# IQTLabs/WITW

Measured on AMD Instinct MI355X. Metric: image-pairs/sec (embedding+similarity), higher is better.
Workload: dtype f32

## Files before the change

include/witw_hip.h:

```cpp
#ifndef WITW_HIP_H
#define WITW_HIP_H

#ifdef __cplusplus
extern "C" {
#endif

const char* witw_last_error(void);
int witw_version(void);
int witw_device_check(int device);
const char* witw_last_kernel_variant(void);
const char* witw_last_conv_form(void);


int witw_conv3x3_tile_n(int cout);
int witw_conv3x3_workgroup_waves(int B, int H, int W, int Cout, int stride_h);
long long witw_conv3x3_packed_floats(int cout, int cin);
int witw_conv3x3_bias_floats(int cout);
int witw_conv3x3_pack_weights(const float* w_kcrs, float* wpk, int cout, int cin, int transpose_flip, void* stream);
int witw_nchw_to_nhwc8(const float* x, float* y, int B, int C, int H, int W, void* stream);
int witw_conv3x3_fwd(const float* x, const float* wpk, const float* bias, const float* dropmask, float* y, int B, int H,
                     int W, int Cin, int Cout, int stride_h, int pad_circular, int relu, int pool, int out_nchw,
                     void* stream);

int witw_conv3x3_first_pack(const float* w, float* wf, int C, int round_bf16, void* stream);
int witw_conv_first2_bf16_fwd(const float* x, const void* wf0, const float* bias0, const void* wpk2, const float* bias2, void* y,
                              int B, int C, int H, int W, int pad_circular, void* stream);
int witw_conv_first2_bf16_fwd_train(const float* x, const void* wf0, const float* bias0, const void* wpk2, const float* bias2, void* y,
                                    unsigned char* pool_code, unsigned char* gate_bits, int B, int C, int H, int W, int pad_circular,
                                    void* stream);
int witw_conv3x3_bf16_gatebits_ok(int B, int H, int W, int Cin, int Cout);
int witw_conv3x3_bf16_fwd_gatebits(const void* x_bf16, const void* wpk_bf16, const float* bias, const void* gate_bits, void* y, int B, int H,
                                   int W, int Cin, int Cout, int pad_circular, int relu, void* stream);
int witw_conv3x3_first_fwd(const float* x, const float* wf, const float* bias, void* y, int B, int C, int H, int W,
                           int pad_circular, int relu, int out_bf16, void* stream);

int witw_conv3x3_fwd_ex(const float* x, const float* wpk, const float* bias, const float* dropmask, const float* gate,
                        const float* post_scale, const float* post_shift, float* y, unsigned char* pool_code, int B, int H,
                        int W, int Cin, int Cout, int stride_h, int pad_circular, int relu, float lrelu_slope, int pool,
                        int out_nchw, int dilate_h, void* stream);
int witw_conv3x3_dil_skip(int enable);
long long witw_conv3x3_packed_floats_wino(int cout, int cin);
int witw_conv3x3_pack_weights_wino(const float* w_kcrs, float* wpk_wino, int cout, int cin, void* stream);
int witw_conv3x3_fwd_wino(const float* x, const float* wpk, const float* wpk_wino, const float* bias, const float* dropmask,
                          const float* gate, const float* post_scale, const float* post_shift, float* y, unsigned char* pool_code,
                          int B, int H, int W, int Cin, int Cout, int stride_h, int pad_circular, int relu, float lrelu_slope,
                          int pool, int out_nchw, int dilate_h, void* stream);
int witw_conv3x3_wino(int enable);
int witw_maxpool2x2_bwd(const float* dy, const unsigned char* pool_code, float* dx, int B, int Hp, int Wp, int H, int W,
                        int C, void* stream);
int witw_nchw_to_nhwc(const float* x, float* y, int B, int C, int H, int W, int Cpad, void* stream);
int witw_conv3x3_wgrad_splits(int B, int Ho, int Wo, int Cin, int Cout);
long long witw_conv3x3_wgrad_workspace_floats(int B, int H, int W, int Cin, int Cout, int stride_h);
int witw_conv3x3_wgrad(const float* x, const float* dz, float* dw, float* db, float* workspace, int B, int H, int W, int Cin,
                       int cin_real, int Cout, int stride_h, int pad_circular, int accumulate, void* stream);
int witw_adam_step(float* param, const float* grad, float* exp_avg, float* exp_avg_sq, long long n, float lr, float beta1,
                   float beta2, float eps, int step, void* stream);
int witw_adam_step_multi(float* const* param, const float* const* grad, float* const* exp_avg, float* const* exp_avg_sq,
                         const long long* n, const int* step, int count, float lr, float beta1, float beta2, float eps, void* stream);

long long witw_match_workspace_floats(int Bo, int Bs);
int witw_match_fwd(const float* ov, const float* su, int Bo, int Bs, int We, long long* orientation, float* distance,
                   float* score, float* workspace, void* stream);
int witw_match_fwd_masked(const float* ov, const float* su, int Bo, int Bs, int We, long long* orientation, float* distance,
                          float* score, float* workspace, const unsigned long long* shift_mask, void* stream);
long long witw_match_fixed_workspace_floats(int Bo, int Bs);
int witw_match_fwd_fixed(const float* ov, const float* su, int Bo, int Bs, int We, const long long* shift ,
                         long long* orientation, float* distance, float* score, float* workspace, void* stream);
long long witw_match_spectrum_floats(long long n_embeddings);
int witw_match_spectrum(const float* emb, float* spec, int B, int W, int role ,
                        void* stream);
long long witw_match_dft_workspace_floats(int Bo, int Bs);
int witw_match_fwd_dft(const float* ov, const float* su, const float* spec_ov, const float* spec_su, int Bo, int Bs, int We,
                       long long* orientation, float* distance, float* score, float* workspace, void* stream);
int witw_match_fwd_dft_gap(const float* ov, const float* su, const float* spec_ov, const float* spec_su, int Bo, int Bs, int We,
                           long long* orientation, float* distance, float* score, float* gap, float* workspace, void* stream);
int witw_match_fwd_dft_masked(const float* ov, const float* su, const float* spec_ov, const float* spec_su, int Bo, int Bs, int We,
                              long long* orientation, float* distance, float* score, float* gap , float* workspace,
                              const unsigned long long* shift_mask, void* stream);
long long witw_match_bwd_scratch_floats(int Bo, int Bs, int We);
int witw_match_bwd(const float* ov, const float* su, const long long* orientation, const float* score, const float* workspace,
                   const float* grad_distance, float* grad_ov, float* grad_su, float* scratch, int Bo, int Bs, int We,
                   void* stream);
int witw_crop_overhead(const float* ov, const long long* orientation, float* out , int Bo, int Bs,
                       int We, void* stream);
int witw_l2_distance(const float* cropped , const float* su , float* distance, int Bo, int Bs, int n,
                     void* stream);
int witw_rank_count(const float* distance , int* ranks , int Bo, int Bs, int true_offset, void* stream);

int witw_topk_smallest(const float* distance, float* values, long long* indices, int Bo, int Bs, int k, long long row_offset,
                       void* stream);
long long witw_topk_workspace_bytes(int Bo, int Bs, int k);
int witw_topk_smallest_ws(const float* distance, float* values, long long* indices, int Bo, int Bs, int k, long long row_offset,
                          void* workspace, void* stream);
int witw_topk_smallest_after(const float* distance, float* values, long long* indices, int Bo, int Bs, int k, long long row_offset,
                             const float* after_value, const long long* after_index, void* workspace, void* stream);
int witw_rank_count_thresh(const float* distance, const float* threshold, int* ranks, int Bo, int Bs, void* stream);

int witw_match_pairs(const float* ov, const float* su, const float* wn, const float* sn, const int* pair_o, const int* pair_s,
                     int n_pairs, int Bo, int Bs, int We, long long* orientation, float* distance, float* score, void* stream);
int witw_rank_count_band(const float* distance, const float* threshold, float eps, int* counts, int* pair_o, int* pair_s,
// ... 184 lines not shown
```

witw_amd/_lib.py:

```python
import ctypes
import os
from ctypes import c_char_p, c_float, c_int, c_longlong, c_void_p

from . import build as _build

_LIB = None
_GUARDS = None

SIGNATURES = {
    'witw_last_error': (c_char_p, []),
    'witw_version': (c_int, []),
    'witw_last_kernel_variant': (c_char_p, []),
    'witw_last_conv_form': (c_char_p, []),
    'witw_device_check': (c_int, [c_int]),
    'witw_conv3x3_tile_n': (c_int, [c_int]),
    'witw_conv3x3_workgroup_waves': (c_int, [c_int] * 5),
    'witw_conv3x3_packed_floats': (c_longlong, [c_int, c_int]),
    'witw_conv3x3_bias_floats': (c_int, [c_int]),
    'witw_conv3x3_pack_weights': (c_int, [c_void_p, c_void_p, c_int, c_int, c_int, c_void_p]),
    'witw_nchw_to_nhwc8': (c_int, [c_void_p, c_void_p, c_int, c_int, c_int, c_int, c_void_p]),
    'witw_conv3x3_fwd': (c_int, [c_void_p, c_void_p, c_void_p, c_void_p, c_void_p] + [c_int] * 10 + [c_void_p]),
    'witw_conv3x3_fwd_ex': (c_int, [c_void_p] * 9 + [c_int] * 8 + [c_float] + [c_int] * 3 + [c_void_p]),
    'witw_conv3x3_dil_skip': (c_int, [c_int]),
    'witw_conv3x3_packed_floats_wino': (c_longlong, [c_int, c_int]),
    'witw_conv3x3_pack_weights_wino': (c_int, [c_void_p, c_void_p, c_int, c_int, c_void_p]),
    'witw_conv3x3_fwd_wino': (c_int, [c_void_p] * 10 + [c_int] * 8 + [c_float] + [c_int] * 3 + [c_void_p]),
    'witw_conv3x3_wino': (c_int, [c_int]),
    'witw_maxpool2x2_bwd': (c_int, [c_void_p, c_void_p, c_void_p] + [c_int] * 6 + [c_void_p]),
    'witw_conv3x3_packed_floats_taps4': (c_longlong, [c_int, c_int]),
    'witw_conv3x3_pack_weights_taps4': (c_int, [c_void_p, c_void_p, c_int, c_int, c_int, c_void_p]),
    'witw_conv3x3_fwd_taps4': (c_int, [c_void_p] * 7 + [c_int] * 6 + [c_float, c_int, c_void_p]),
    'witw_conv3x3_taps4_ksplit': (c_int, [c_int] * 5),
    'witw_conv3x3_fwd_taps4_ex': (c_int, [c_void_p] * 7 + [c_int] * 6 + [c_float] + [c_int] * 5 + [c_void_p]),
    'witw_conv3x3_wgrad_taps4': (c_int, [c_void_p] * 5 + [c_int] * 7 + [c_void_p]),
    'witw_nchw_to_nhwc': (c_int, [c_void_p, c_void_p, c_int, c_int, c_int, c_int, c_int, c_void_p]),
    'witw_conv3x3_wgrad_splits': (c_int, [c_int] * 5),
    'witw_conv3x3_wgrad_workspace_floats': (c_longlong, [c_int] * 6),
    'witw_conv3x3_wgrad': (c_int, [c_void_p] * 5 + [c_int] * 9 + [c_void_p]),
    'witw_adam_step': (c_int, [c_void_p, c_void_p, c_void_p, c_void_p, c_longlong, c_float, c_float, c_float, c_float, c_int,
                               c_void_p]),
    'witw_adam_step_multi': (c_int, [c_void_p] * 6 + [c_int, c_float, c_float, c_float, c_float, c_void_p]),
    'witw_conv3x3_first_pack': (c_int, [c_void_p, c_void_p, c_int, c_int, c_void_p]),
    'witw_conv3x3_first_fwd': (c_int, [c_void_p, c_void_p, c_void_p, c_void_p] + [c_int] * 7 + [c_void_p]),
    'witw_conv3x3_bf16_mfma16': (c_int, [c_int]),
    'witw_conv3x3_bf16_wres': (c_int, [c_int]),
    'witw_conv3x3_bf16_packed_elems': (c_longlong, [c_int, c_int]),
    'witw_conv3x3_bf16_pack_weights': (c_int, [c_void_p, c_void_p, c_int, c_int, c_void_p]),
    'witw_conv3x3_bf16_pack_weights_ex': (c_int, [c_void_p, c_void_p, c_int, c_int, c_int, c_void_p]),
    'witw_conv3x3_bf16_pack_weights_multi': (c_int, [c_void_p] * 7 + [c_int, c_void_p]),
    'witw_nchw_f32_to_nhwc_bf16': (c_int, [c_void_p, c_void_p] + [c_int] * 5 + [c_void_p]),
    'witw_conv3x3_bf16_fwd': (c_int, [c_void_p] * 4 + [c_int] * 10 + [c_void_p]),
    'witw_conv3x3_bf16_fwd_ex': (c_int, [c_void_p] * 7 + [c_int] * 11 + [c_void_p]),
    'witw_maxpool2x2_bwd_bf16': (c_int, [c_void_p] * 3 + [c_int] * 6 + [c_void_p]),
    'witw_octet_elems': (c_longlong, [c_int] * 4),
    'witw_nhwc_bf16_to_octet': (c_int, [c_void_p, c_void_p] + [c_int] * 4 + [c_void_p]),
    'witw_conv3x3_wgrad_bf16_workspace_floats': (c_longlong, [c_int] * 6),
    'witw_conv3x3_wgrad_bf16': (c_int, [c_void_p] * 5 + [c_int] * 9 + [c_void_p]),
    'witw_conv3x3_wgrad_bf16_nhwc_workspace_floats': (c_longlong, [c_int] * 6),
    'witw_conv3x3_wgrad_bf16_mfma16': (c_int, [c_int]),
    'witw_conv3x3_wgrad_bf16_nhwc': (c_int, [c_void_p] * 5 + [c_int] * 9 + [c_void_p]),
    'witw_conv3x3_f16x3_packed_elems': (c_longlong, [c_int, c_int]),
    'witw_conv3x3_f16x3_pack_weights': (c_int, [c_void_p, c_void_p, c_int, c_int, c_void_p]),
    'witw_nchw_f32_to_split_f16': (c_int, [c_void_p, c_void_p] + [c_int] * 5 + [c_void_p]),
    'witw_split_f16_to_f32': (c_int, [c_void_p, c_void_p, c_longlong, c_int, c_void_p]),
    'witw_conv3x3_f16x3_fwd': (c_int, [c_void_p] * 4 + [c_int] * 10 + [c_void_p]),
    'witw_conv3x3_f16x3_pack_weights_ex': (c_int, [c_void_p, c_void_p, c_int, c_int, c_int, c_void_p]),
    'witw_conv3x3_f16x3_fwd_ex': (c_int, [c_void_p] * 8 + [c_int] * 11 + [c_void_p]),
    'witw_maxpool2x2_bwd_split': (c_int, [c_void_p] * 3 + [c_int] * 6 + [c_void_p]),
    'witw_octet_split_elems': (c_longlong, [c_int] * 4),
    'witw_split_f16_to_octet': (c_int, [c_void_p, c_void_p] + [c_int] * 4 + [c_void_p]),
    'witw_conv3x3_wgrad_f16x3_workspace_floats': (c_longlong, [c_int] * 6),
    'witw_conv3x3_wgrad_f16x3': (c_int, [c_void_p] * 6 + [c_int] * 9 + [c_void_p]),
    'witw_conv4x4s2_first_fwd': (c_int, [c_void_p] * 6 + [c_int] * 5 + [c_float, c_void_p]),
    'witw_space_to_depth2': (c_int, [c_void_p, c_void_p] + [c_int] * 9 + [c_void_p, c_void_p, c_void_p]),
    'witw_space_to_depth2_mosaic': (c_int, [c_void_p, c_void_p] + [c_int] * 5 + [c_void_p]),
    'witw_taps4_splitk_finish': (c_int, [c_void_p, c_int, c_void_p, c_int, c_float] + [c_void_p] * 3 + [c_int] * 7 + [c_void_p]),
    'witw_gem_pool': (c_int, [c_void_p, c_void_p] + [c_int] * 8 + [c_float, c_void_p, c_void_p, c_void_p]),
    'witw_bn_workspace_floats': (c_longlong, [c_int] * 4),
    'witw_bn_train_stats': (c_int, [c_void_p] + [c_int] * 6 + [c_void_p, c_void_p, c_float, c_float] + [c_void_p] * 8),
    'witw_bn_lrelu_bwd': (c_int, [c_void_p] * 8 + [c_int] * 6 + [c_float, c_void_p, c_void_p]),
# ... 135 lines not shown
```

witw_amd/csrc/conv3x3.hip:

```cpp
#include "common.h"
#include <stdlib.h>
#include <algorithm>

namespace {

constexpr int TW_WIDE = 64;

__device__ const f32x4 g_zero_f4[1] = {{0.f, 0.f, 0.f, 0.f}};

struct ConvArgs {
    const float* x;
    const float* wpk;
    const float* bias;
    const float* dropmask;
    const float* post_scale;
    const float* post_shift;
    float lrelu;
    unsigned char* pool_code;
    const float* gate;
    float* y;
    int B, H, W, Cin, Cout;
    int Ho, Wo;
    int tiles_x, tiles_y;
    int n_tiles, sp_total, sp_per_xcd, xcd_map;
    int circ, relu, out_nchw;
    int force_nw;
    int force_geo;
    int dil_h;
    int tap_base;
    int ksplit, kc_per_split;
    size_t split_stride;
    int s2d, s2d_h, s2d_w, valid_h, valid_w;
    int wino;
    const float* wpk_wino;
#ifdef WITW_STAMPS
    unsigned long long* stamps;
#endif
};

template <int NW, bool POOL>
__device__ __forceinline__ void conv_wino_h2(const ConvArgs& p, f32x4* smem) {
    constexpr int TH = NW, TW = 64, IW = TW + 2, IH = TH + 2;
    constexpr int NTHREADS = 64 * NW;
    constexpr int WTN = 64;
    constexpr int IN_F4 = 2 * IH * IW;
    constexpr int W_F4 = 12 * 2 * WTN;
    constexpr int STAGE_F4 = IN_F4 + W_F4;
    constexpr int NIN = (IN_F4 + NTHREADS - 1) / NTHREADS;
    constexpr int NWT = W_F4 / NTHREADS;
    static_assert(NWT * NTHREADS == W_F4, "the filter slab splits evenly over the workgroup");

    const int tid = threadIdx.x;
    const int lane = tid & 63;
    const int wave = tid >> 6;
    const int l31 = lane & 31;
    const int hq = lane >> 5;

    int ntile, sp;
    if (p.xcd_map) {
        const int g = blockIdx.x >> 3;
        ntile = g % p.n_tiles;
        sp = (blockIdx.x & 7) * p.sp_per_xcd + g / p.n_tiles;
        if (sp >= p.sp_total) return;
    } else {
        ntile = blockIdx.x / p.sp_total;
        sp = blockIdx.x - ntile * p.sp_total;
    }
    const int tiles_img = p.tiles_x * p.tiles_y;
    const int b = sp / tiles_img;
    sp -= b * tiles_img;
    const int ty = sp / p.tiles_x;
    const int tx = sp - ty * p.tiles_x;
    const int oy0 = ty * TH;
    const int ox0 = tx * TW;
    const int n0 = ntile * WTN;
    const int nkc = p.Cin >> 3;

    constexpr unsigned OOR = 0x80000000u;
    const size_t img_floats = (size_t)p.H * p.W * p.Cin;
    __amdgpu_buffer_rsrc_t in_rs = __builtin_amdgcn_make_buffer_rsrc((void*)(p.x + (size_t)b * img_floats), 0,
                                                                     (unsigned)(img_floats * 4), 0x00020000);
    __amdgpu_buffer_rsrc_t w_rs = __builtin_amdgcn_make_buffer_rsrc(
        (void*)(reinterpret_cast<const f32x4*>(p.wpk_wino) + (size_t)ntile * nkc * W_F4), 0, (unsigned)nkc * W_F4 * 16u, 0x00020000);
    unsigned gin[NIN];
#pragma unroll
    for (int i = 0; i < NIN; ++i) {
        const int s = tid + i * NTHREADS;
        const int pix = s >> 1, q = s & 1;
        const int r = pix / IW, c = pix - r * IW;
        const int gr = oy0 - 1 + r;
        int gc = ox0 - 1 + c;
        bool ok = (s < IN_F4) && gr >= 0 && gr < p.H;
        if (p.circ) {
            gc %= p.W;
            if (gc < 0) gc += p.W;
        } else {
            ok = ok && gc >= 0 && gc < p.W;
        }
        gin[i] = ok ? (unsigned)((((size_t)gr * p.W + gc) * p.Cin + q * 4) * 4) : OOR;
    }
    const unsigned gwoff = (unsigned)tid * 16u;
    f32x4 rin[NIN], rw[NWT];
    auto load_one = [&](int kc, int i) {
        if (i < NIN) rin[i] = __builtin_bit_cast(f32x4, __builtin_amdgcn_raw_buffer_load_b128(in_rs, gin[i], (unsigned)kc * 32u, 0));
        else rw[i - NIN] = __builtin_bit_cast(f32x4, __builtin_amdgcn_raw_buffer_load_b128(
                 w_rs, gwoff, (unsigned)kc * W_F4 * 16u + (unsigned)(i - NIN) * (NTHREADS * 16u), 0));
    };
    auto store_one = [&](int buf, int i) {
        f32x4* in_s = smem + buf * STAGE_F4;
        if (i < NIN) {
            const int s = tid + i * NTHREADS;
            f32x4* dst = (NIN * NTHREADS == IN_F4 || s < IN_F4) ? in_s + (s & 1) * (IH * IW) + (s >> 1) : smem + 2 * STAGE_F4;
            *dst = rin[i];
        } else {
            in_s[IN_F4 + tid + (i - NIN) * NTHREADS] = rw[i - NIN];
        }
    };

    const int wm = wave >> 1, wn = wave & 1;
    const int abase = hq * (IH * IW) + 2 * wm * IW + l31;
    const int wbase = hq * WTN + wn * 32 + l31;
    f32x16 acc[4][2];
#pragma unroll
    for (int t = 0; t < 4; ++t)
#pragma unroll
        for (int ct = 0; ct < 2; ++ct)
#pragma unroll
            for (int r = 0; r < 16; ++r) acc[t][ct][r] = 0.f;

    f32x4 fa[2][4], fb[2][4];
    auto read_a = [&](int set, const f32x4* in_s, int s, int i) { fa[set][i] = in_s[abase + i * IW + 32 * (s & 1) + (s >> 1)]; };
    auto read_b = [&](int set, const f32x4* w_s, int kw, int t) { fb[set][t] = w_s[(kw * 4 + t) * 2 * WTN + wbase]; };
    auto transform2 = [&](int set, int k) {
        const int j = k >> 1;
        const float d0 = fa[set][0][j], d1 = fa[set][1][j], d2 = fa[set][2][j], d3 = fa[set][3][j];
        if ((k & 1) == 0) {
            fa[set][0][j] = d0 - d2;
            fa[set][3][j] = d1 - d3;
        } else {
            fa[set][1][j] = d1 + d2;
            fa[set][2][j] = d2 - d1;
        }
    };
    auto mfma_one = [&](int set, int bset, int ct, int i) {
        const int j = i >> 2, t = i & 3;
        acc[t][ct] = __builtin_amdgcn_mfma_f32_32x32x2f32(fa[set][t][j], fb[bset][t][j], acc[t][ct], 0, 0, 0);
    };

#pragma unroll
    for (int i = 0; i < NIN + NWT; ++i) load_one(0, i);
#pragma unroll
    for (int i = 0; i < NIN + NWT; ++i) store_one(0, i);
    __syncthreads();
#pragma unroll
    for (int i = 0; i < 4; ++i) read_b(0, smem + IN_F4, 0, i);
    __builtin_amdgcn_sched_barrier(0);
#pragma unroll
    for (int i = 0; i < 4; ++i) read_a(0, smem, 0, i);
#pragma unroll
    for (int k = 0; k < 8; ++k) transform2(0, k);

    auto step = [&](int set, int bset, int ct, auto&& mem, bool barrier_mid) {
#pragma unroll
        for (int i = 0; i < 16; ++i) {
            mfma_one(set, bset, ct, i);
            mem(i);
            if (i >= 8) transform2(set ^ 1, i - 8);
            __builtin_amdgcn_sched_barrier(0);
            if (barrier_mid && i == 7) {
                __syncthreads();
                __builtin_amdgcn_sched_barrier(0);
            }
        }
    };
    static_assert(16 - 6 - (NIN + NWT) >= 0, "step too short to hide the staging instructions");

    for (int kc = 0; kc < nkc; ++kc) {
        const int cur = kc & 1;
        const int kn = (kc + 1 < nkc) ? kc + 1 : kc;
        const f32x4* in_s = smem + cur * STAGE_F4;
        const f32x4* w_s = in_s + IN_F4;
        const f32x4* in_n = smem + (cur ^ 1) * STAGE_F4;
        step(0, 0, 0, [&](int i) {
            if (i < 4) read_a(1, in_s, 1, i);
            else if (i < 6) read_b(1, w_s, 1, i - 4);
            else if (i < 6 + NIN + NWT) load_one(kn, i - 6);
        }, false);
        step(1, 0, 1, [&](int i) {
            if (i < 4) read_a(0, in_s, 2, i);
            else if (i < 6) read_b(1, w_s, 1, i - 2);
        }, false);
        step(0, 1, 0, [&](int i) {
            if (i < 4) read_a(1, in_s, 3, i);
            else if (i < 8) read_b(0, w_s, 2, i - 4);
        }, false);
        step(1, 1, 1, [&](int i) {
            if (i < 4) read_a(0, in_s, 4, i);
            else if (i < 4 + NIN + NWT) store_one(cur ^ 1, i - 4);
        }, false);
        step(0, 0, 0, [&](int i) {
            if (i < 4) read_a(1, in_s, 5, i);
        }, true);
        step(1, 0, 1, [&](int i) {
            if (i < 4) read_a(0, in_n, 0, i);
            else if (i < 8) read_b(1, in_n + IN_F4, 0, i - 4);
        }, false);
#pragma unroll
        for (int t = 0; t < 4; ++t) fb[0][t] = fb[1][t];
    }

    f32x16 yv[2][2];
#pragma unroll
    for (int ct = 0; ct < 2; ++ct)
#pragma unroll
        for (int r = 0; r < 16; ++r) {
            const float m0 = acc[0][ct][r], m1 = acc[1][ct][r], m2 = acc[2][ct][r], m3 = acc[3][ct][r];
            yv[0][ct][r] = (m0 + m1) + m2;
            yv[1][ct][r] = (m1 - m2) - m3;
        }
    const int nb = n0 + wn * 32;
    const int nch = nb + l31;
    const float bv = p.bias[nch];
    const float dm = (p.dropmask != nullptr && nch < p.Cout) ? p.dropmask[(size_t)b * p.Cout + nch] : 1.f;
    const int act = p.relu;
    auto fin = [&](float v) {
        v = (v + bv) * dm;
        if (act == 1) v = fmaxf(v, 0.f);
        else if (act == 2) v = v > 0.f ? v : v * p.lrelu;
        return v;
    };
    const int Hy = POOL ? (p.Ho >> 1) : p.Ho;
    const int Wy = POOL ? (p.Wo >> 1) : p.Wo;
    float* slab = reinterpret_cast<float*>(smem) + wave * (32 * 32);
    const int prow = lane >> 3, pc4 = (lane & 7) * 4;
    if constexpr (!POOL) {
#pragma unroll
        for (int k = 0; k < 2; ++k)
#pragma unroll
            for (int ct = 0; ct < 2; ++ct) {
#pragma unroll
                for (int r = 0; r < 16; ++r) slab[((r & 3) + 8 * (r >> 2) + 4 * hq) * 32 + l31] = fin(yv[k][ct][r]);
                const int yy = oy0 + 2 * wm + k;
#pragma unroll
                for (int g = 0; g < 4; ++g) {
                    const int m = g * 8 + prow;
                    const f32x4 v = *reinterpret_cast<const f32x4*>(slab + m * 32 + pc4);
                    const int xx = ox0 + 32 * ct + m;
                    if (yy < Hy && xx < Wy && nb + pc4 < p.Cout)
                        __builtin_nontemporal_store(v, reinterpret_cast<f32x4*>(p.y + (((size_t)b * Hy + yy) * Wy + xx) * p.Cout + nb + pc4));
                }
            }
    } else {
        const int yy = (oy0 + 2 * wm) >> 1;
#pragma unroll
        for (int ct = 0; ct < 2; ++ct)
#pragma unroll
            for (int g = 0; g < 4; ++g)
#pragma unroll
                for (int e = 0; e < 2; ++e) {
                    const int r = 4 * g + 2 * e;
                    const float a00 = yv[0][ct][r], a01 = yv[0][ct][r + 1], a10 = yv[1][ct][r], a11 = yv[1][ct][r + 1];
                    const float m = fmaxf(fmaxf(a00, a01), fmaxf(a10, a11));
                    const int pc = 16 * ct + 4 * g + 2 * hq + e;
                    slab[pc * 32 + l31] = fin(m);
                    const int xx = (ox0 >> 1) + pc;
                    if (p.pool_code != nullptr && yy < Hy && xx < Wy && nch < p.Cout) {
                        const int code = (a00 == m) ? 0 : (a01 == m) ? 1 : (a10 == m) ? 2 : 3;
                        p.pool_code[(((size_t)b * Hy + yy) * Wy + xx) * p.Cout + nch] = (unsigned char)code;
                    }
                }
#pragma unroll
        for (int g = 0; g < 4; ++g) {
            const int pc = g * 8 + prow;
            const f32x4 v = *reinterpret_cast<const f32x4*>(slab + pc * 32 + pc4);
            const int xx = (ox0 >> 1) + pc;
            if (yy < Hy && xx < Wy && nb + pc4 < p.Cout)
                __builtin_nontemporal_store(v, reinterpret_cast<f32x4*>(p.y + (((size_t)b * Hy + yy) * Wy + xx) * p.Cout + nb + pc4));
        }
    }
}

template <int TN, int SH, bool POOL, int NW, int GEO, int TAPS = 9>
__global__ __launch_bounds__(64 * NW) void conv3x3_nhwc_f32_kernel(ConvArgs p) {
    static_assert(TAPS == 9 || TAPS == 4, "3x3 window or a 2x2 sub-window");
    constexpr bool NARROW = GEO == 1;
    constexpr bool DIL = GEO == 2;
    static_assert(!DIL || (TN == 128 && NW == 8 && SH == 1 && TAPS == 9 && !POOL), "the dilated form exists for the 8-wave 128-channel tile");
    constexpr int TH = NARROW ? 4 * NW : NW;
    constexpr int TW = NARROW ? 16 : 64;
    constexpr int IW = TW + 2;
    constexpr int NTHREADS = 64 * NW;
    constexpr int IH = (TH - 1) * SH + 3;
    constexpr int IN_F4 = 2 * IH * IW;
    constexpr int W_F4 = TAPS * 2 * TN;
    constexpr int STAGE_F4 = IN_F4 + W_F4;
    constexpr int NIN = (IN_F4 + NTHREADS - 1) / NTHREADS;
    constexpr int NWT = (W_F4 + NTHREADS - 1) / NTHREADS;
    constexpr int WGM = (TN == 128) ? NW / 2 : NW;
    constexpr int WM = (2 * NW) / WGM;
    constexpr int WN = 2;

    constexpr bool WINO = SH == 1 && TAPS == 9 && GEO == 0 && (TN == 128 || POOL);
    constexpr int WINO_F4 = WINO ? 2 * (2 * (NW + 2) * IW + 12 * 2 * 64) + 1 : 0;
    constexpr int DIRECT_F4 = (2 * STAGE_F4 + 1 > NW * 512) ? 2 * STAGE_F4 + 1 : NW * 512;
    constexpr int SMEM_F4 = DIRECT_F4 > WINO_F4 ? DIRECT_F4 : WINO_F4;
    __shared__ f32x4 smem[SMEM_F4];
    static_assert(SMEM_F4 * 16 >= NW * 32 * 64 * 4, "the buffer must hold one epilogue slab per wave");
    if constexpr (WINO) {
        if (p.wino) {
            conv_wino_h2<NW, POOL>(p, smem);
            return;
        }
    }

    const int tid = threadIdx.x;
    const int lane = tid & 63;
    const int wave = tid >> 6;
    const int l31 = lane & 31;
    const int hq = lane >> 5;

    int ntile, sp;
    if (p.xcd_map) {
        const int g = blockIdx.x >> 3;
        ntile = g % p.n_tiles;
        sp = (blockIdx.x & 7) * p.sp_per_xcd + g / p.n_tiles;
        if (sp >= p.sp_total) return;
    } else {
        ntile = blockIdx.x / p.sp_total;
        sp = blockIdx.x - ntile * p.sp_total;
    }
    const int tiles_img = p.tiles_x * p.tiles_y;
    const int b = sp / tiles_img;
    sp -= b * tiles_img;
    const int ty = sp / p.tiles_x;
    const int tx = sp - ty * p.tiles_x;
    const int oy0 = ty * TH;
    const int ox0 = tx * TW;
    const int n0 = ntile * TN;
    int nkc = p.Cin >> 3;
    int kc_lo = 0;
    if constexpr (TAPS == 4) {
        if (p.ksplit > 1) {
            kc_lo = (int)blockIdx.y * p.kc_per_split;
            nkc = min(nkc - kc_lo, p.kc_per_split);
        }
    }

    constexpr unsigned OOR = 0x80000000u;
    const int Hp = p.dil_h ? (p.H - 1) / 2 + 1 : p.H;
    const size_t img_floats = (size_t)Hp * p.W * p.Cin;
    __amdgpu_buffer_rsrc_t in_rs = __builtin_amdgcn_make_buffer_rsrc(
        (void*)(p.x + (size_t)b * img_floats + (size_t)kc_lo * 8), 0, (unsigned)(img_floats * 4) - (unsigned)kc_lo * 32u, 0x00020000);
    const unsigned wtile_bytes = (unsigned)nkc * W_F4 * 16u;
    __amdgpu_buffer_rsrc_t w_rs = __builtin_amdgcn_make_buffer_rsrc(
        (void*)(reinterpret_cast<const f32x4*>(p.wpk) + ((size_t)ntile * (p.Cin >> 3) + kc_lo) * W_F4), 0, wtile_bytes, 0x00020000);
    unsigned gin[NIN];
#pragma unroll
    for (int i = 0; i < NIN; ++i) {
        const int s = tid + i * NTHREADS;
        const int pix = s >> 1, q = s & 1;
        const int r = pix / IW, c = pix - r * IW;
        const int gr = oy0 * SH - 1 + r;
// ... 419 lines not shown
                v[j] = w[(((size_t)ci * src_cin + co) * 3 + (2 - kh)) * 3 + (2 - kw)];
        }
    }
    reinterpret_cast<f32x4*>(wpk)[idx] = v;
}

__global__ void pack_weights_wino_kernel(const float* __restrict__ w, float* __restrict__ wpk, int Cout, int Cin, int nkc,
                                         size_t total) {
    const size_t idx = (size_t)blockIdx.x * blockDim.x + threadIdx.x;
    if (idx >= total) return;
    size_t t = idx;
    const int n = t % 64; t /= 64;
    const int q = t % 2; t /= 2;
    const int tr = t % 4; t /= 4;
    const int kw = t % 3; t /= 3;
    const int kc = t % nkc; t /= nkc;
    const int co = (int)t * 64 + n;
    f32x4 v = {0.f, 0.f, 0.f, 0.f};
#pragma unroll
    for (int j = 0; j < 4; ++j) {
        const int ci = kc * 8 + q * 4 + j;
        if (co < Cout && ci < Cin) {
            const float* g = w + ((size_t)co * Cin + ci) * 9 + kw;
            const float g0 = g[0], g1 = g[3], g2 = g[6];
            v[j] = tr == 0 ? g0 : tr == 1 ? ((g0 + g1) + g2) * 0.5f : tr == 2 ? ((g0 - g1) + g2) * 0.5f : g2;
        }
    }
    reinterpret_cast<f32x4*>(wpk)[idx] = v;
}

__global__ void nchw_to_nhwc8_kernel(const float* __restrict__ x, float* __restrict__ y, int B, int C, int H, int W) {
    const size_t npix = (size_t)B * H * W;
    const size_t idx = (size_t)blockIdx.x * blockDim.x + threadIdx.x;
    if (idx >= npix) return;
    const size_t hw = (size_t)H * W;
    const size_t b = idx / hw, r = idx - b * hw;
    float v[8];
#pragma unroll
    for (int c = 0; c < 8; ++c) v[c] = (c < C) ? x[(b * C + c) * hw + r] : 0.f;
    f32x4* o = reinterpret_cast<f32x4*>(y + idx * 8);
    o[0] = f32x4{v[0], v[1], v[2], v[3]};
    o[1] = f32x4{v[4], v[5], v[6], v[7]};
}

__global__ void nchw_to_nhwc_kernel(const float* __restrict__ x, float* __restrict__ y, int C, int Cp, size_t hw, size_t total) {
    const size_t idx = (size_t)blockIdx.x * blockDim.x + threadIdx.x;
    if (idx >= total) return;
    const int c = idx % Cp;
    const size_t t = idx / Cp;
    const size_t b = t / hw, r = t - b * hw;
    y[idx] = (c < C) ? x[(b * C + c) * hw + r] : 0.f;
}

template <int TN, int SH, bool POOL, int NW, int GEO, int TAPS = 9>
int launch_conv_nw(ConvArgs a, hipStream_t st) {
    a.tiles_y = cdiv(a.Ho, GEO == 1 ? 4 * NW : NW);
    a.tiles_x = cdiv(a.Wo, GEO == 1 ? 16 : 64);
    const long long sp_total = (long long)a.B * a.tiles_x * a.tiles_y;
    a.n_tiles = cdiv(a.Cout, a.wino ? 64 : TN);
    a.sp_per_xcd = (int)((sp_total + 7) / 8);
    if (sp_total < 8) a.xcd_map = 0;
    const long long grid = a.xcd_map ? 8LL * a.sp_per_xcd * a.n_tiles : sp_total * a.n_tiles;
    if (grid <= 0 || grid > 0x7fffffffLL || sp_total > 0x7fffffffLL) {
        witw_set_error("conv3x3: grid %lld out of range", grid);
        return WITW_ERR_INVALID;
    }
    a.sp_total = (int)sp_total;
    const unsigned gy = (TAPS == 4 && a.ksplit > 1) ? (unsigned)a.ksplit : 1u;
    hipLaunchKernelGGL((conv3x3_nhwc_f32_kernel<TN, SH, POOL, NW, GEO, TAPS>), dim3((unsigned)grid, gy), dim3(64 * NW), 0, st, a);
    WITW_CHECK_LAUNCH("conv3x3_nhwc_f32");
    witw_note_variant("conv3x3_nhwc_f32_kernel<%d,%d,%s,%d,%d,%d>", TN, SH, POOL ? "true" : "false", NW, GEO, TAPS);
    if (a.wino) witw_note_conv_form("wino_h2");
    return WITW_OK;
}

int choose_waves(int B, int Ho, int Wo, int Cout, int force_nw) {
    const int TN = (Cout >= 128) ? 128 : 64;
    const long long big = (long long)cdiv(Cout, TN) * B * cdiv(Wo, TW_WIDE) * cdiv(Ho, 8);
    if (force_nw == 4) return 4;
    return (force_nw == 8 || ((Ho % 8) == 0 && witw_fills_rounds(big))) ? 8 : 4;
}

bool choose_narrow(int Wo, int force_geo) { return force_geo == 1 || (force_geo != 0 && Wo <= 32); }

int env_int(const char* name, int dflt) {
    const char* e = getenv(name);
    return e ? atoi(e) : dflt;
}

int g_dil_skip = -1;
int dil_skip() {
    if (g_dil_skip < 0) {
        const char* e = getenv("WITW_CONV_DILSKIP");
        g_dil_skip = e ? (atoi(e) != 0) : 1;
    }
    return g_dil_skip;
}

int g_wino = -1;
int wino_on() {
    if (g_wino < 0) {
        const char* e = getenv("WITW_CONV_WINO");
        g_wino = e ? (atoi(e) != 0) : 1;
    }
    return g_wino;
}

template <int TN, int SH, bool POOL>
int launch_conv(ConvArgs a, hipStream_t st) {
    const bool wino = SH == 1 && (TN == 128 || POOL) && a.wpk_wino != nullptr && wino_on() && a.gate == nullptr && !a.dil_h &&
                      !a.out_nchw && a.post_scale == nullptr && (a.Cout & 3) == 0 && a.force_geo != 1 &&
                      !choose_narrow(a.Wo, a.force_geo);
    a.wino = wino ? 1 : 0;
    if (wino) return choose_waves(a.B, a.Ho, a.Wo, a.Cout, a.force_nw) == 8 ? launch_conv_nw<TN, SH, POOL, 8, 0>(a, st)
                                                                          : launch_conv_nw<TN, SH, POOL, 4, 0>(a, st);
#ifndef WITW_NO_NARROW
    if (choose_narrow(a.Wo, a.force_geo)) return launch_conv_nw<TN, SH, POOL, 4, 1>(a, st);
#endif
    if (choose_waves(a.B, a.Ho, a.Wo, a.Cout, a.force_nw) == 8) {
        if constexpr (TN == 128 && SH == 1 && !POOL) {
            if (a.dil_h && dil_skip()) return launch_conv_nw<TN, SH, POOL, 8, 2>(a, st);
        }
        return launch_conv_nw<TN, SH, POOL, 8, 0>(a, st);
    }
    return launch_conv_nw<TN, SH, POOL, 4, 0>(a, st);
}

template <int TN>
int launch_conv_taps4(const ConvArgs& a, hipStream_t st) {
#ifndef WITW_NO_NARROW
    if (choose_narrow(a.Wo, a.force_geo)) return launch_conv_nw<TN, 1, false, 4, 1, 4>(a, st);
#endif
    if (choose_waves(a.B, a.Ho, a.Wo, a.Cout, a.force_nw) == 8) return launch_conv_nw<TN, 1, false, 8, 0, 4>(a, st);
    return launch_conv_nw<TN, 1, false, 4, 0, 4>(a, st);
}

}

#ifdef WITW_STAMPS
unsigned long long* witw_conv_stamps_ptr = nullptr;
#endif

extern "C" {

int witw_conv3x3_tile_n(int cout) { return cout >= 128 ? 128 : 64; }

int witw_conv3x3_workgroup_waves(int B, int H, int W, int Cout, int stride_h) {
    if (B <= 0 || H <= 0 || W <= 0 || Cout <= 0 || (stride_h != 1 && stride_h != 2)) return -1;
    if (choose_narrow(W, env_int("WITW_CONV_GEO", -1))) return 4;
    return choose_waves(B, (H + 2 - 3) / stride_h + 1, W, Cout, env_int("WITW_CONV_NW", 0));
}

long long witw_conv3x3_packed_floats(int cout, int cin) {
    if (cout <= 0 || cin <= 0) return -1;
    const int TN = witw_conv3x3_tile_n(cout);
    const long long n_tiles = cdiv(cout, TN), nkc = cdiv(cin, 8);
    return n_tiles * nkc * 9 * 2 * TN * 4;
}
// ... 153 lines not shown
    a.post_scale = post_scale; a.post_shift = post_shift; a.lrelu = lrelu_slope;
    a.pool_code = pool ? pool_code : nullptr;
    a.B = B; a.H = H; a.W = W; a.Cin = Cin; a.Cout = Cout;
    a.Ho = (H + 2 - 3) / stride_h + 1;
    a.Wo = W;
    a.tiles_x = 0;
    a.tiles_y = 0;
    a.force_nw = env_int("WITW_CONV_NW", 0);
    a.force_geo = env_int("WITW_CONV_GEO", -1);
    a.xcd_map = env_int("WITW_CONV_XCD", 1) != 0;
    a.circ = pad_circular; a.relu = relu; a.out_nchw = out_nchw; a.dil_h = dilate_h; a.tap_base = 0;
    a.ksplit = 1; a.kc_per_split = 0; a.split_stride = 0; a.s2d = 0; a.s2d_h = a.s2d_w = a.valid_h = a.valid_w = 0;
    a.wino = 0; a.wpk_wino = wpk_wino;
#ifdef WITW_STAMPS
    a.stamps = witw_conv_stamps_ptr;
#endif
    hipStream_t st = (hipStream_t)stream;
    const int TN = witw_conv3x3_tile_n(Cout);
    if (TN == 128) {
        if (stride_h == 2) return launch_conv<128, 2, false>(a, st);
        return pool ? launch_conv<128, 1, true>(a, st) : launch_conv<128, 1, false>(a, st);
    }
    if (stride_h == 2) return launch_conv<64, 2, false>(a, st);
    return pool ? launch_conv<64, 1, true>(a, st) : launch_conv<64, 1, false>(a, st);
}

}

extern "C" {

int witw_conv3x3_fwd_ex(const float* x, const float* wpk, const float* bias, const float* dropmask, const float* gate,
                        const float* post_scale, const float* post_shift, float* y, unsigned char* pool_code, int B, int H,
                        int W, int Cin, int Cout, int stride_h, int pad_circular, int relu, float lrelu_slope, int pool,
                        int out_nchw, int dilate_h, void* stream) {
    return conv3x3_fwd_any(x, wpk, nullptr, bias, dropmask, gate, post_scale, post_shift, y, pool_code, B, H, W, Cin, Cout,
                           stride_h, pad_circular, relu, lrelu_slope, pool, out_nchw, dilate_h, stream);
}

int witw_conv3x3_fwd_wino(const float* x, const float* wpk, const float* wpk_wino, const float* bias, const float* dropmask,
                          const float* gate, const float* post_scale, const float* post_shift, float* y, unsigned char* pool_code,
                          int B, int H, int W, int Cin, int Cout, int stride_h, int pad_circular, int relu, float lrelu_slope,
                          int pool, int out_nchw, int dilate_h, void* stream) {
    WITW_CHECK_ARG(wpk_wino, "conv3x3_fwd_wino: null Winograd filter");
    return conv3x3_fwd_any(x, wpk, wpk_wino, bias, dropmask, gate, post_scale, post_shift, y, pool_code, B, H, W, Cin, Cout,
                           stride_h, pad_circular, relu, lrelu_slope, pool, out_nchw, dilate_h, stream);
}

int witw_conv3x3_wino(int enable) {
    const int prev = wino_on();
    if (enable >= 0) g_wino = enable != 0;
    return prev;
}

long long witw_conv3x3_packed_floats_wino(int cout, int cin) {
    if (cout <= 0 || cin <= 0) return -1;
    return (long long)cdiv(cout, 64) * cdiv(cin, 8) * 12 * 2 * 64 * 4;
}

int witw_conv3x3_pack_weights_wino(const float* w_kcrs, float* wpk_wino, int cout, int cin, void* stream) {
    WITW_CHECK_ARG(w_kcrs && wpk_wino, "pack_weights_wino: null pointer");
    WITW_CHECK_ARG(cout > 0 && cin > 0, "pack_weights_wino: bad shape cout=%d cin=%d", cout, cin);
    const int n_tiles = cdiv(cout, 64), nkc = cdiv(cin, 8);
    const size_t total = (size_t)n_tiles * nkc * 12 * 2 * 64;
    hipLaunchKernelGGL(pack_weights_wino_kernel, dim3((unsigned)((total + 255) / 256)), dim3(256), 0, (hipStream_t)stream,
                       w_kcrs, wpk_wino, cout, cin, nkc, total);
    WITW_CHECK_LAUNCH("pack_weights_wino");
    return WITW_OK;
}

int witw_conv3x3_dil_skip(int enable) {
    const int prev = dil_skip();
    if (enable >= 0) g_dil_skip = enable != 0;
    return prev;
}

int witw_conv3x3_fwd(const float* x, const float* wpk, const float* bias, const float* dropmask, float* y, int B, int H,
                     int W, int Cin, int Cout, int stride_h, int pad_circular, int relu, int pool, int out_nchw,
                     void* stream) {
    return witw_conv3x3_fwd_ex(x, wpk, bias, dropmask, nullptr, nullptr, nullptr, y, nullptr, B, H, W, Cin, Cout, stride_h,
                               pad_circular, relu ? 1 : 0, 0.f, pool, out_nchw, 0, stream);
}

}
```

witw_amd/ops.py:

```python
import torch

from . import _lib


PROFILE = None
PROFILE_BY_KERNEL = None


def _stream():
    return torch.cuda.current_stream().cuda_stream


def _dev_f32(t, name):
    if not (isinstance(t, torch.Tensor) and t.is_cuda):
        raise _lib.WitwError('%s must be a CUDA(HIP) tensor: the WITW hot path has no CPU fallback' % name)
    if t.dtype != torch.float32:
        raise _lib.WitwError('%s must be float32, got %s' % (name, t.dtype))
    if not t.is_contiguous():
        raise _lib.WitwError('%s must be contiguous' % name)
    return t


def _p(t):
    return 0 if t is None else t.data_ptr()
# ... 1209 lines not shown
    _lib.check(lib.witw_space_to_depth2(x.data_ptr(), y.data_ptr(), B, Hp, Wp, H, W, C, cpad, int(in_nchw), int(normalize),
                                        _p(scale), _p(shift), _stream()), 'witw_space_to_depth2')
    return y


def gem_pool(x_nhwc, valid_hw, out, col0, p=3., scale=None, shift=None):
    lib = _lib.load()
    x = _dev_f32(x_nhwc, 'x')
    B, Hp, Wp, C = x.shape
    H, W = valid_hw
    _lib.check(lib.witw_gem_pool(x.data_ptr(), out.data_ptr(), B, Hp, Wp, H, W, C, out.shape[1], col0, float(p), _p(scale),
                                 _p(shift), _stream()), 'witw_gem_pool')
    return out


def embed_normalize_(f):
    lib = _lib.load()
    f = _dev_f32(f, 'f')
    _lib.check(lib.witw_embed_normalize(f.data_ptr(), f.shape[0], f.shape[1], _stream()), 'witw_embed_normalize')
    return f


def pairwise_sqdist(a, b, take_sqrt=False):
    lib = _lib.load()
    a, b = _dev_f32(a, 'a'), _dev_f32(b, 'b')
    if a.dim() != 2 or b.dim() != 2 or a.shape[1] != b.shape[1]:
        raise _lib.WitwError('pairwise_sqdist: need [Na,n] and [Nb,n]')
    D = torch.empty((a.shape[0], b.shape[0]), dtype=torch.float32, device=a.device)
    _lib.check(lib.witw_pairwise_sqdist(a.data_ptr(), b.data_ptr(), D.data_ptr(), a.shape[0], b.shape[0], a.shape[1],
                                        int(take_sqrt), _stream()), 'witw_pairwise_sqdist')
    return D


def exhaustive_triplet_loss(D, soft_margin=False, alpha=10., margin=1.):
    lib = _lib.load()
    D = _dev_f32(D, 'D')
    B = D.shape[0]
    loss = torch.empty((1,), dtype=torch.float32, device=D.device)
    ws = torch.empty((B,), dtype=torch.float32, device=D.device)
    _lib.check(lib.witw_exhaustive_triplet_loss(D.data_ptr(), B, int(soft_margin), float(alpha), float(margin),
                                                loss.data_ptr(), ws.data_ptr(), _stream()), 'witw_exhaustive_triplet_loss')
    return loss.reshape(())


def last_conv_form():
    v = _lib.load().witw_last_conv_form()
    return v.decode() if v else ''


def conv_wino(enable=None):
    return bool(_lib.load().witw_conv3x3_wino(-1 if enable is None else int(bool(enable))))


def last_kernel_variant():
    v = _lib.load().witw_last_kernel_variant()
    return v.decode() if v else ''


def bf16_mfma16(enable=None):
    return bool(_lib.load().witw_conv3x3_bf16_mfma16(-1 if enable is None else int(bool(enable))))


def bf16_wres(enable=None):
    return bool(_lib.load().witw_conv3x3_bf16_wres(-1 if enable is None else int(bool(enable))))


class PackedConvBf16(_Packed):
    CPAD, DTYPE = 16, torch.bfloat16

    def __init__(self, weight, bias, transpose_flip=False, reuse=None):
        lib = _lib.load()
        w, reuse = self._filter_buffer(weight, transpose_flip, reuse, lib.witw_conv3x3_bf16_packed_elems)
        _lib.check(lib.witw_conv3x3_bf16_pack_weights_ex(w.data_ptr(), self.wpk.data_ptr(), self.cout, self.cin,
                                                         int(bool(transpose_flip)), _stream()), 'witw_conv3x3_bf16_pack_weights_ex')
        self._bias_buffer(reuse, bias)

    @classmethod
    def batch(cls, items):
        import ctypes
        lib = _lib.load()
        out, tab = [], []
        for weight, bias, transpose_flip, reuse in items:
            pk = cls.__new__(cls)
            w, reuse = pk._filter_buffer(weight, transpose_flip, reuse, lib.witw_conv3x3_bf16_packed_elems)
            pk._bias_buffer(reuse)
            b = None if bias is None else _dev_f32(bias.detach(), 'bias')
            if b is not None and b.numel() != pk.cout:
                raise _lib.WitwError('PackedConvBf16.batch: bias of %d elements for %d output channels' % (b.numel(), pk.cout))
            tab.append((w, pk.wpk, b, pk.bias, pk.cout, pk.cin, int(bool(transpose_flip))))
            out.append(pk)
        k = len(tab)
        if k:
            vp = ctypes.c_void_p
            _lib.check(lib.witw_conv3x3_bf16_pack_weights_multi(
                (vp * k)(*[t[0].data_ptr() for t in tab]), (vp * k)(*[t[1].data_ptr() for t in tab]),
                (vp * k)(*[None if t[2] is None else t[2].data_ptr() for t in tab]), (vp * k)(*[t[3].data_ptr() for t in tab]),
                (ctypes.c_int * k)(*[t[4] for t in tab]), (ctypes.c_int * k)(*[t[5] for t in tab]),
                (ctypes.c_int * k)(*[t[6] for t in tab]), k, _stream()), 'witw_conv3x3_bf16_pack_weights_multi')
        return out


def nchw_to_nhwc_bf16(x, cpad=16):
    lib = _lib.load()
    x = _dev_f32(x, 'x')
    B, C, H, W = x.shape
    y = torch.empty((B, H, W, cpad), dtype=torch.bfloat16, device=x.device)
# ... 291 lines not shown
```

Baseline: 2491.

## Make Winograd conv kernel persistent and prefetch next tile during epilogue

The Winograd 3x3 conv path now launches at most one workgroup per CU, and each workgroup loops over several output tiles. The first input/filter chunk of the next tile is staged before the current tile's epilogue runs, so loads overlap with output writes, and the epilogue slab moves to its own shared-memory region so it no longer clobbers the staging buffers. This is meant to remove per-workgroup launch and prologue costs and pipeline-fill bubbles between tiles. In exchange it uses more shared memory, which can lower occupancy, and running only one workgroup per CU limits latency hiding.

Measured after the change: 2537 (median of 6 runs). 1.02x the previous value.

```diff
diff --git a/include/witw_hip.h b/include/witw_hip.h
--- a/include/witw_hip.h
+++ b/include/witw_hip.h
@@ -46,6 +46,7 @@
                           int B, int H, int W, int Cin, int Cout, int stride_h, int pad_circular, int relu, float lrelu_slope,
                           int pool, int out_nchw, int dilate_h, void* stream);
 int witw_conv3x3_wino(int enable);
+int witw_conv3x3_wino_run(int enable);
 int witw_maxpool2x2_bwd(const float* dy, const unsigned char* pool_code, float* dx, int B, int Hp, int Wp, int H, int W,
                         int C, void* stream);
 int witw_nchw_to_nhwc(const float* x, float* y, int B, int C, int H, int W, int Cpad, void* stream);
diff --git a/witw_amd/_lib.py b/witw_amd/_lib.py
--- a/witw_amd/_lib.py
+++ b/witw_amd/_lib.py
@@ -26,6 +26,7 @@
     'witw_conv3x3_pack_weights_wino': (c_int, [c_void_p, c_void_p, c_int, c_int, c_void_p]),
     'witw_conv3x3_fwd_wino': (c_int, [c_void_p] * 10 + [c_int] * 8 + [c_float] + [c_int] * 3 + [c_void_p]),
     'witw_conv3x3_wino': (c_int, [c_int]),
+    'witw_conv3x3_wino_run': (c_int, [c_int]),
     'witw_maxpool2x2_bwd': (c_int, [c_void_p, c_void_p, c_void_p] + [c_int] * 6 + [c_void_p]),
     'witw_conv3x3_packed_floats_taps4': (c_longlong, [c_int, c_int]),
     'witw_conv3x3_pack_weights_taps4': (c_int, [c_void_p, c_void_p, c_int, c_int, c_int, c_void_p]),
diff --git a/witw_amd/csrc/conv3x3.hip b/witw_amd/csrc/conv3x3.hip
--- a/witw_amd/csrc/conv3x3.hip
+++ b/witw_amd/csrc/conv3x3.hip
@@ -33,6 +33,7 @@
     int s2d, s2d_h, s2d_w, valid_h, valid_w;
     int wino;
     const float* wpk_wino;
+    int wino_items, wino_wgs;
 #ifdef WITW_STAMPS
     unsigned long long* stamps;
 #endif
@@ -50,55 +51,73 @@
     constexpr int NWT = W_F4 / NTHREADS;
     static_assert(NWT * NTHREADS == W_F4, "the filter slab splits evenly over the workgroup");
 
-    const int tid = threadIdx.x;
+    int tid = threadIdx.x;
+    asm volatile("" : "+v"(tid));
     const int lane = tid & 63;
     const int wave = tid >> 6;
     const int l31 = lane & 31;
     const int hq = lane >> 5;
 
-    int ntile, sp;
-    if (p.xcd_map) {
-        const int g = blockIdx.x >> 3;
-        ntile = g % p.n_tiles;
-        sp = (blockIdx.x & 7) * p.sp_per_xcd + g / p.n_tiles;
-        if (sp >= p.sp_total) return;
-    } else {
-        ntile = blockIdx.x / p.sp_total;
-        sp = blockIdx.x - ntile * p.sp_total;
-    }
     const int tiles_img = p.tiles_x * p.tiles_y;
-    const int b = sp / tiles_img;
-    sp -= b * tiles_img;
-    const int ty = sp / p.tiles_x;
-    const int tx = sp - ty * p.tiles_x;
-    const int oy0 = ty * TH;
-    const int ox0 = tx * TW;
-    const int n0 = ntile * WTN;
+    auto item_sp = [&](int it, int& ntile) {
+        if (p.xcd_map) {
+            const int g = it >> 3;
+            ntile = g % p.n_tiles;
+            return (it & 7) * p.sp_per_xcd + g / p.n_tiles;
+        }
+        ntile = it / p.sp_total;
+        return it - ntile * p.sp_total;
+    };
+    auto step_item = [&](int it) { return p.wino_items - it > p.wino_wgs ? it + p.wino_wgs : p.wino_items; };
+    auto next_item = [&](int it) {
+        int nt;
+        while (it < p.wino_items && item_sp(it, nt) >= p.sp_total) it = step_item(it);
+        return it;
+    };
+    int it = next_item(blockIdx.x);
+    if (it >= p.wino_items) return;
     const int nkc = p.Cin >> 3;
 
     constexpr unsigned OOR = 0x80000000u;
     const size_t img_floats = (size_t)p.H * p.W * p.Cin;
-    __amdgpu_buffer_rsrc_t in_rs = __builtin_amdgcn_make_buffer_rsrc((void*)(p.x + (size_t)b * img_floats), 0,
-                                                                     (unsigned)(img_floats * 4), 0x00020000);
-    __amdgpu_buffer_rsrc_t w_rs = __builtin_amdgcn_make_buffer_rsrc(
-        (void*)(reinterpret_cast<const f32x4*>(p.wpk_wino) + (size_t)ntile * nkc * W_F4), 0, (unsigned)nkc * W_F4 * 16u, 0x00020000);
+    int ntile, b, oy0, ox0;
+    __amdgpu_buffer_rsrc_t in_rs, w_rs;
     unsigned gin[NIN];
-#pragma unroll
-    for (int i = 0; i < NIN; ++i) {
-        const int s = tid + i * NTHREADS;
-        const int pix = s >> 1, q = s & 1;
-        const int r = pix / IW, c = pix - r * IW;
-        const int gr = oy0 - 1 + r;
-        int gc = ox0 - 1 + c;
-        bool ok = (s < IN_F4) && gr >= 0 && gr < p.H;
-        if (p.circ) {
-            gc %= p.W;
-            if (gc < 0) gc += p.W;
-        } else {
-            ok = ok && gc >= 0 && gc < p.W;
-        }
-        gin[i] = ok ? (unsigned)((((size_t)gr * p.W + gc) * p.Cin + q * 4) * 4) : OOR;
-    }
+    auto decode = [&](int item, int& nt_, int& b_, int& oy0_, int& ox0_) {
+        int sp = item_sp(item, nt_);
+        b_ = sp / tiles_img;
+        sp -= b_ * tiles_img;
+        const int ty = sp / p.tiles_x;
+        oy0_ = ty * TH;
+        ox0_ = (sp - ty * p.tiles_x) * TW;
+    };
+    auto stage_from = [&](int nt_, int b_, int oy0_, int ox0_, bool live) {
+        in_rs = __builtin_amdgcn_make_buffer_rsrc((void*)(p.x + (size_t)b_ * img_floats), 0, live ? (unsigned)(img_floats * 4) : 0u,
+                                                  0x00020000);
+        w_rs = __builtin_amdgcn_make_buffer_rsrc((void*)(reinterpret_cast<const f32x4*>(p.wpk_wino) + (size_t)nt_ * nkc * W_F4), 0,
+                                                 live ? (unsigned)nkc * W_F4 * 16u : 0u, 0x00020000);
+        if (!live) return;
+        int t = tid;
+        asm volatile("" : "+v"(t));
+#pragma unroll
+        for (int i = 0; i < NIN; ++i) {
+            const int s = t + i * NTHREADS;
+            const int pix = s >> 1, q = s & 1;
+            const int r = pix / IW, c = pix - r * IW;
+            const int gr = oy0_ - 1 + r;
+            int gc = ox0_ - 1 + c;
+            bool ok = (s < IN_F4) && gr >= 0 && gr < p.H;
+            if (p.circ) {
+                gc %= p.W;
+                if (gc < 0) gc += p.W;
+            } else {
+                ok = ok && gc >= 0 && gc < p.W;
+            }
+            gin[i] = ok ? (unsigned)((((size_t)gr * p.W + gc) * p.Cin + q * 4) * 4) : OOR;
+        }
+    };
+    decode(it, ntile, b, oy0, ox0);
+    stage_from(ntile, b, oy0, ox0, true);
     const unsigned gwoff = (unsigned)tid * 16u;
     f32x4 rin[NIN], rw[NWT];
     auto load_one = [&](int kc, int i) {
@@ -175,9 +194,7 @@
     };
     static_assert(16 - 6 - (NIN + NWT) >= 0, "step too short to hide the staging instructions");
 
-    for (int kc = 0; kc < nkc; ++kc) {
-        const int cur = kc & 1;
-        const int kn = (kc + 1 < nkc) ? kc + 1 : kc;
+    auto chunk = [&](int cur, int kn) __attribute__((always_inline)) {
         const f32x4* in_s = smem + cur * STAGE_F4;
         const f32x4* w_s = in_s + IN_F4;
         const f32x4* in_n = smem + (cur ^ 1) * STAGE_F4;
@@ -207,76 +224,104 @@
         }, false);
 #pragma unroll
         for (int t = 0; t < 4; ++t) fb[0][t] = fb[1][t];
-    }
-
-    f32x16 yv[2][2];
-#pragma unroll
-    for (int ct = 0; ct < 2; ++ct)
-#pragma unroll
-        for (int r = 0; r < 16; ++r) {
-            const float m0 = acc[0][ct][r], m1 = acc[1][ct][r], m2 = acc[2][ct][r], m3 = acc[3][ct][r];
-            yv[0][ct][r] = (m0 + m1) + m2;
-            yv[1][ct][r] = (m1 - m2) - m3;
-        }
-    const int nb = n0 + wn * 32;
-    const int nch = nb + l31;
-    const float bv = p.bias[nch];
-    const float dm = (p.dropmask != nullptr && nch < p.Cout) ? p.dropmask[(size_t)b * p.Cout + nch] : 1.f;
-    const int act = p.relu;
-    auto fin = [&](float v) {
-        v = (v + bv) * dm;
-        if (act == 1) v = fmaxf(v, 0.f);
-        else if (act == 2) v = v > 0.f ? v : v * p.lrelu;
-        return v;
-    };
+    };
+
     const int Hy = POOL ? (p.Ho >> 1) : p.Ho;
     const int Wy = POOL ? (p.Wo >> 1) : p.Wo;
-    float* slab = reinterpret_cast<float*>(smem) + wave * (32 * 32);
+    float* slab = reinterpret_cast<float*>(smem + 2 * STAGE_F4 + 1) + wave * (32 * 32);
     const int prow = lane >> 3, pc4 = (lane & 7) * 4;
-    if constexpr (!POOL) {
-#pragma unroll
-        for (int k = 0; k < 2; ++k)
-#pragma unroll
-            for (int ct = 0; ct < 2; ++ct) {
-#pragma unroll
-                for (int r = 0; r < 16; ++r) slab[((r & 3) + 8 * (r >> 2) + 4 * hq) * 32 + l31] = fin(yv[k][ct][r]);
-                const int yy = oy0 + 2 * wm + k;
-#pragma unroll
-                for (int g = 0; g < 4; ++g) {
-                    const int m = g * 8 + prow;
-                    const f32x4 v = *reinterpret_cast<const f32x4*>(slab + m * 32 + pc4);
-                    const int xx = ox0 + 32 * ct + m;
-                    if (yy < Hy && xx < Wy && nb + pc4 < p.Cout)
-                        __builtin_nontemporal_store(v, reinterpret_cast<f32x4*>(p.y + (((size_t)b * Hy + yy) * Wy + xx) * p.Cout + nb + pc4));
-                }
+    int cur = 0;
+    for (;;) {
+        for (int kc = 1; kc < nkc; ++kc) {
+            chunk(cur, kc);
+            cur ^= 1;
+        }
+        const int it_n = next_item(step_item(it));
+        const bool more = it_n < p.wino_items;
+        int ntile_n = ntile, b_n = b, oy0_n = oy0, ox0_n = ox0;
+        if (more) decode(it_n, ntile_n, b_n, oy0_n, ox0_n);
+        stage_from(ntile_n, b_n, oy0_n, ox0_n, more);
+        chunk(cur, 0);
+        cur ^= 1;
+
+        const int n0 = ntile * WTN;
+        f32x16 yv[2][2];
+#pragma unroll
+        for (int ct = 0; ct < 2; ++ct)
+#pragma unroll
+            for (int r = 0; r < 16; ++r) {
+                const float m0 = acc[0][ct][r], m1 = acc[1][ct][r], m2 = acc[2][ct][r], m3 = acc[3][ct][r];
+                yv[0][ct][r] = (m0 + m1) + m2;
+                yv[1][ct][r] = (m1 - m2) - m3;
             }
-    } else {
-        const int yy = (oy0 + 2 * wm) >> 1;
-#pragma unroll
-        for (int ct = 0; ct < 2; ++ct)
-#pragma unroll
-            for (int g = 0; g < 4; ++g)
-#pragma unroll
-                for (int e = 0; e < 2; ++e) {
-                    const int r = 4 * g + 2 * e;
-                    const float a00 = yv[0][ct][r], a01 = yv[0][ct][r + 1], a10 = yv[1][ct][r], a11 = yv[1][ct][r + 1];
-                    const float m = fmaxf(fmaxf(a00, a01), fmaxf(a10, a11));
-                    const int pc = 16 * ct + 4 * g + 2 * hq + e;
-                    slab[pc * 32 + l31] = fin(m);
-                    const int xx = (ox0 >> 1) + pc;
-                    if (p.pool_code != nullptr && yy < Hy && xx < Wy && nch < p.Cout) {
-                        const int code = (a00 == m) ? 0 : (a01 == m) ? 1 : (a10 == m) ? 2 : 3;
-                        p.pool_code[(((size_t)b * Hy + yy) * Wy + xx) * p.Cout + nch] = (unsigned char)code;
+        const int nb = n0 + wn * 32;
+        const int nch = nb + l31;
+        const float bv = p.bias[nch];
+        const float dm = (p.dropmask != nullptr && nch < p.Cout) ? p.dropmask[(size_t)b * p.Cout + nch] : 1.f;
+        const int act = p.relu;
+        auto fin = [&](float v) {
+            v = (v + bv) * dm;
+            if (act == 1) v = fmaxf(v, 0.f);
+            else if (act == 2) v = v > 0.f ? v : v * p.lrelu;
+            return v;
+        };
+        if constexpr (!POOL) {
+#pragma unroll
+            for (int k = 0; k < 2; ++k)
+#pragma unroll
+                for (int ct = 0; ct < 2; ++ct) {
+#pragma unroll
+                    for (int r = 0; r < 16; ++r) slab[((r & 3) + 8 * (r >> 2) + 4 * hq) * 32 + l31] = fin(yv[k][ct][r]);
+                    const int yy = oy0 + 2 * wm + k;
+#pragma unroll
+                    for (int g = 0; g < 4; ++g) {
+                        const int m = g * 8 + prow;
+                        const f32x4 v = *reinterpret_cast<const f32x4*>(slab + m * 32 + pc4);
+                        const int xx = ox0 + 32 * ct + m;
+                        if (yy < Hy && xx < Wy && nb + pc4 < p.Cout)
+                            __builtin_nontemporal_store(v, reinterpret_cast<f32x4*>(p.y + (((size_t)b * Hy + yy) * Wy + xx) * p.Cout + nb + pc4));
                     }
                 }
-#pragma unroll
-        for (int g = 0; g < 4; ++g) {
-            const int pc = g * 8 + prow;
-            const f32x4 v = *reinterpret_cast<const f32x4*>(slab + pc * 32 + pc4);
-            const int xx = (ox0 >> 1) + pc;
-            if (yy < Hy && xx < Wy && nb + pc4 < p.Cout)
-                __builtin_nontemporal_store(v, reinterpret_cast<f32x4*>(p.y + (((size_t)b * Hy + yy) * Wy + xx) * p.Cout + nb + pc4));
-        }
+        } else {
+            const int yy = (oy0 + 2 * wm) >> 1;
+#pragma unroll
+            for (int ct = 0; ct < 2; ++ct)
+#pragma unroll
+                for (int g = 0; g < 4; ++g)
+#pragma unroll
+                    for (int e = 0; e < 2; ++e) {
+                        const int r = 4 * g + 2 * e;
+                        const float a00 = yv[0][ct][r], a01 = yv[0][ct][r + 1], a10 = yv[1][ct][r], a11 = yv[1][ct][r + 1];
+                        const float m = fmaxf(fmaxf(a00, a01), fmaxf(a10, a11));
+                        const int pc = 16 * ct + 4 * g + 2 * hq + e;
+                        slab[pc * 32 + l31] = fin(m);
+                        const int xx = (ox0 >> 1) + pc;
+                        if (p.pool_code != nullptr && yy < Hy && xx < Wy && nch < p.Cout) {
+                            const int code = (a00 == m) ? 0 : (a01 == m) ? 1 : (a10 == m) ? 2 : 3;
+                            p.pool_code[(((size_t)b * Hy + yy) * Wy + xx) * p.Cout + nch] = (unsigned char)code;
+                        }
+                    }
+#pragma unroll
+            for (int g = 0; g < 4; ++g) {
+                const int pc = g * 8 + prow;
+                const f32x4 v = *reinterpret_cast<const f32x4*>(slab + pc * 32 + pc4);
+                const int xx = (ox0 >> 1) + pc;
+                if (yy < Hy && xx < Wy && nb + pc4 < p.Cout)
+                    __builtin_nontemporal_store(v, reinterpret_cast<f32x4*>(p.y + (((size_t)b * Hy + yy) * Wy + xx) * p.Cout + nb + pc4));
+            }
+        }
+        if (!more) break;
+        it = it_n;
+        ntile = ntile_n;
+        b = b_n;
+        oy0 = oy0_n;
+        ox0 = ox0_n;
+#pragma unroll
+        for (int t = 0; t < 4; ++t)
+#pragma unroll
+            for (int ct = 0; ct < 2; ++ct)
+#pragma unroll
+                for (int r = 0; r < 16; ++r) acc[t][ct][r] = 0.f;
     }
 }
 
@@ -301,13 +346,13 @@
     constexpr int WN = 2;
 
     constexpr bool WINO = SH == 1 && TAPS == 9 && GEO == 0 && (TN == 128 || POOL);
-    constexpr int WINO_F4 = WINO ? 2 * (2 * (NW + 2) * IW + 12 * 2 * 64) + 1 : 0;
+    constexpr int WINO_F4 = WINO ? 2 * (2 * (NW + 2) * IW + 12 * 2 * 64) + 1 + NW * 256 : 0;
     constexpr int DIRECT_F4 = (2 * STAGE_F4 + 1 > NW * 512) ? 2 * STAGE_F4 + 1 : NW * 512;
     constexpr int SMEM_F4 = DIRECT_F4 > WINO_F4 ? DIRECT_F4 : WINO_F4;
     __shared__ f32x4 smem[SMEM_F4];
     static_assert(SMEM_F4 * 16 >= NW * 32 * 64 * 4, "the buffer must hold one epilogue slab per wave");
     if constexpr (WINO) {
-        if (p.wino) {
+        if (__builtin_expect(p.wino != 0, 0)) {
             conv_wino_h2<NW, POOL>(p, smem);
             return;
         }
@@ -833,6 +878,9 @@
     y[idx] = (c < C) ? x[(b * C + c) * hw + r] : 0.f;
 }
 
+int env_int(const char* name, int dflt);
+int wino_run();
+
 template <int TN, int SH, bool POOL, int NW, int GEO, int TAPS = 9>
 int launch_conv_nw(ConvArgs a, hipStream_t st) {
     a.tiles_y = cdiv(a.Ho, GEO == 1 ? 4 * NW : NW);
@@ -848,7 +896,14 @@
     }
     a.sp_total = (int)sp_total;
     const unsigned gy = (TAPS == 4 && a.ksplit > 1) ? (unsigned)a.ksplit : 1u;
-    hipLaunchKernelGGL((conv3x3_nhwc_f32_kernel<TN, SH, POOL, NW, GEO, TAPS>), dim3((unsigned)grid, gy), dim3(64 * NW), 0, st, a);
+    a.wino_items = (int)grid;
+    a.wino_wgs = (int)grid;
+    if (a.wino && wino_run()) {
+        const int forced = env_int("WITW_CONV_WINO_WGS", 0);
+        a.wino_wgs = (int)std::min<long long>(grid, forced > 0 ? forced : witw_cu_count());
+    }
+    hipLaunchKernelGGL((conv3x3_nhwc_f32_kernel<TN, SH, POOL, NW, GEO, TAPS>), dim3(a.wino ? (unsigned)a.wino_wgs : (unsigned)grid, gy),
+                       dim3(64 * NW), 0, st, a);
     WITW_CHECK_LAUNCH("conv3x3_nhwc_f32");
     witw_note_variant("conv3x3_nhwc_f32_kernel<%d,%d,%s,%d,%d,%d>", TN, SH, POOL ? "true" : "false", NW, GEO, TAPS);
     if (a.wino) witw_note_conv_form("wino_h2");
@@ -885,6 +940,15 @@
         g_wino = e ? (atoi(e) != 0) : 1;
     }
     return g_wino;
+}
+
+int g_wino_run = -1;
+int wino_run() {
+    if (g_wino_run < 0) {
+        const char* e = getenv("WITW_CONV_WINO_RUN");
+        g_wino_run = e ? (atoi(e) != 0) : 1;
+    }
+    return g_wino_run;
 }
 
 template <int TN, int SH, bool POOL>
@@ -1144,6 +1208,12 @@
     return prev;
 }
 
+int witw_conv3x3_wino_run(int enable) {
+    const int prev = wino_run();
+    if (enable >= 0) g_wino_run = enable != 0;
+    return prev;
+}
+
 long long witw_conv3x3_packed_floats_wino(int cout, int cin) {
     if (cout <= 0 || cin <= 0) return -1;
     return (long long)cdiv(cout, 64) * cdiv(cin, 8) * 12 * 2 * 64 * 4;
diff --git a/witw_amd/ops.py b/witw_amd/ops.py
--- a/witw_amd/ops.py
+++ b/witw_amd/ops.py
@@ -1285,6 +1285,10 @@
     return bool(_lib.load().witw_conv3x3_wino(-1 if enable is None else int(bool(enable))))
 
 
+def conv_wino_run(enable=None):
+    return bool(_lib.load().witw_conv3x3_wino_run(-1 if enable is None else int(bool(enable))))
+
+
 def last_kernel_variant():
     v = _lib.load().witw_last_kernel_variant()
     return v.decode() if v else ''
```
